# Ighina/MultimodalTopicSegmentation

Measured on NVIDIA B200. Metric: segmented sentences/sec, higher is better.
Workload: dtype f32

## Files before the change

### multimodaltopicsegmentation_b200/csrc/lstm_rec_h3.cu

```cuda
#include <cooperative_groups.h>
#include <cuda_fp16.h>
#include <stdlib.h>

#include "cluster_utils.cuh"
#include "tcgen05_utils.cuh"

namespace cg = cooperative_groups;

namespace mts {

constexpr int HR_NB = 16;
constexpr int HR_SUB_THREADS = 160;
constexpr int HR_EPI = 128;
constexpr int HR_PIECE_BYTES = 4 * HR_NB * 128;
constexpr int HR_B_BYTES = 2 * HR_PIECE_BYTES;
constexpr int HR_ACT_FLOATS = 4 * HR_NB * 32;
constexpr int HR_TMEM_COLS = 512;
constexpr int HR_W2_COL = 128;
constexpr int HR_ACC_COL = 256;
constexpr int HR_SUB_BYTES = 2 * HR_B_BYTES + HR_ACT_FLOATS * 4 + 1024;
constexpr int HR_HEAD_BYTES = 1024;
static_assert(HR_SUB_BYTES % 1024 == 0, "SWIZZLE_128B operand buffers need 1024-byte alignment");
template <int NT>
constexpr int hr_smem() {
  return (HR_HEAD_BYTES + NT * HR_SUB_BYTES + 1024) > 120 * 1024 ? (HR_HEAD_BYTES + NT * HR_SUB_BYTES + 1024) : 120 * 1024;
}

__host__ __device__ constexpr uint32_t idesc_f16(int M, int N) {
  return (1u << 4) | ((uint32_t)(N >> 3) << 17) | ((uint32_t)(M >> 4) << 24);
}

__device__ __forceinline__ uint32_t h2_bits(float first, float second) {
  const __half2 h = __floats2half2_rn(first, second);
  return *reinterpret_cast<const uint32_t *>(&h);
}
__device__ __forceinline__ float2 h2_floats(uint32_t bits) {
  return __half22float2(*reinterpret_cast<const __half2 *>(&bits));
}
__device__ __forceinline__ void st_async_v4u(uint32_t raddr, uint4 v, uint32_t rbar) {
  asm volatile("st.async.weak.shared::cluster.mbarrier::complete_tx::bytes.v4.b32 [%0], {%1, %2, %3, %4}, [%5];" ::"r"(raddr),
               "r"(v.x), "r"(v.y), "r"(v.z), "r"(v.w), "r"(rbar)
               : "memory");
}
__device__ __forceinline__ void tmem_st16u(uint32_t taddr, const uint32_t (&v)[16]) {
  asm volatile(
      "tcgen05.st.sync.aligned.32x32b.x16.b32 [%0], "
      "{%1, %2, %3, %4, %5, %6, %7, %8, %9, %10, %11, %12, %13, %14, %15, %16};" ::"r"(taddr),
      "r"(v[0]), "r"(v[1]), "r"(v[2]), "r"(v[3]), "r"(v[4]), "r"(v[5]), "r"(v[6]), "r"(v[7]), "r"(v[8]), "r"(v[9]), "r"(v[10]),
      "r"(v[11]), "r"(v[12]), "r"(v[13]), "r"(v[14]), "r"(v[15])
      : "memory");
}

__device__ __forceinline__ void umma_f16_ts_p(uint32_t d_tmem, uint32_t a_tmem, uint32_t b_lo, uint32_t b_hi, uint32_t idesc,
                                              uint32_t acc) {
  asm volatile(
      "{\n\t.reg .pred p;\n\t.reg .b64 bd;\n\t"
      "setp.ne.b32 p, %5, 0;\n\t"
      "mov.b64 bd, {%2, %3};\n\t"
      "tcgen05.mma.cta_group::1.kind::f16 [%0], [%1], bd, %4, p;\n\t}" ::"r"(d_tmem),
      "r"(a_tmem), "r"(b_lo), "r"(b_hi), "r"(idesc), "r"(acc)
      : "memory");
}

constexpr int HR_PROF_STEPS = 4, HR_PROF_SLOTS = 16;
__device__ long long *g_hr_prof = nullptr;
#define HR_STAMP(slot)                                                                     \
  do {                                                                                     \
    if (prof && s >= 8 && s < 8 + HR_PROF_STEPS) prof[(s - 8) * HR_PROF_SLOTS + (slot)] = clock64(); \
  } while (0)

template <bool SAVE, int NT, bool BF16>
__global__ void __cluster_dims__(kCluster, 1, 1) __launch_bounds__(HR_SUB_THREADS * NT, 1)
    lstm_fwd_h3_kernel(const float *__restrict__ gx, const float *__restrict__ w_hh, const int32_t *__restrict__ lengths,
                       const int32_t *__restrict__ order, int B, int T, int n_enc, int n_tiles, int ept,
                       float *__restrict__ y, float *__restrict__ gates, float *__restrict__ y_corr) {
  constexpr bool bf16_mode = BF16;
  extern __shared__ uint8_t smem_raw[];
  uint8_t *smem = reinterpret_cast<uint8_t *>((reinterpret_cast<uintptr_t>(smem_raw) + 1023) & ~(uintptr_t)1023);
  const int tid = threadIdx.x, lane = tid & 31;
  const int warp = __shfl_sync(0xffffffffu, tid >> 5, 0);
  const int sub = (NT == 2 && warp >= 5) ? 1 : 0;
  const int wr = warp - 5 * sub;

  float *rscale_s = reinterpret_cast<float *>(smem);
  uint32_t *tmem_slot = reinterpret_cast<uint32_t *>(smem + 512);
  uint8_t *sub_base = smem + HR_HEAD_BYTES + sub * HR_SUB_BYTES;
  uint8_t *bbuf = sub_base;
  float *act = reinterpret_cast<float *>(bbuf + 2 * HR_B_BYTES);
  uint64_t *bars = reinterpret_cast<uint64_t *>(act + HR_ACT_FLOATS);
  uint64_t *h_full = bars;
  uint64_t *acc_full = bars + 16;
  int *len_s = reinterpret_cast<int *>(bars + 18);
  int *bq_s = len_s + HR_NB;

  cg::cluster_group cluster = cg::this_cluster();
  const uint32_t rank = cluster.block_rank();
  const int n_clusters = gridDim.x / kCluster;
  const int groups = (n_tiles + NT - 1) / NT;
  const int n_items = groups * 2 * n_enc;
  const int ycols = n_enc * 2 * kH;

  if (wr == 0 && lane == 0) {
    for (int i = 0; i < 4; ++i) tc::bar_init(tc::s_u32(&h_full[i]), 1);
    tc::bar_init(tc::s_u32(acc_full), 1);
    asm volatile("fence.mbarrier_init.release.cluster;" ::: "memory");
  }
  if (warp == 0) tc::tmem_alloc<HR_TMEM_COLS>(tc::s_u32(tmem_slot));
  tc::tc_fence_before();
  __syncthreads();
  tc::tc_fence_after();
  const uint32_t tmem_base = *tmem_slot;
  const uint32_t acc_col = HR_ACC_COL + 16 * sub;

  uint32_t ph_h = 0, ph_acc = 0;

  const int et = (wr - 1) * 32 + lane;
  const int q = warp & 3;
  const int cj = et & 7, ce = et >> 3;

  int cur_dir = -1, cur_enc = -1;
  long long *prof = (blockIdx.x == 0 && (tid == 0 || tid == 32)) ? g_hr_prof : nullptr;

  for (int item = blockIdx.x / kCluster; item < n_items; item += n_clusters) {
    const int tile = (item % groups) * NT + sub;
    const int dir = (item / groups) & 1;
    const int enc = item / (2 * groups);
    const float *W = w_hh + ((size_t)enc * 2 + dir) * 4 * kH * kH;

    if (dir != cur_dir || enc != cur_enc) {
      if (sub == 0 && wr >= 1) {
        const float *wrow = W + (size_t)(q * kH + rank * kUnits + lane) * kH;
        float mx = 0.0f;
#pragma unroll 8
        for (int i = 0; i < kH / 4; ++i) {
          const float4 x = __ldg(reinterpret_cast<const float4 *>(wrow) + i);
          mx = fmaxf(fmaxf(mx, fmaxf(fabsf(x.x), fabsf(x.y))), fmaxf(fabsf(x.z), fabsf(x.w)));
        }
        const int ex = (int)((__float_as_uint(mx) >> 23) & 0xFFu);
        int sexp = ex == 0 ? 0 : 127 + 13 - ex;
        sexp = sexp > 110 ? 110 : sexp;
        const float sc = __uint_as_float((uint32_t)(127 + sexp) << 23);
        rscale_s[q * 32 + lane] = __uint_as_float((uint32_t)(127 - sexp) << 23);
        const uint32_t trow = tmem_base + ((uint32_t)(q * 32) << 16);
#pragma unroll 1
        for (int kk = 0; kk < 8; ++kk) {
          const int src_blk = ((int)rank - kk) & 7;
          uint32_t w1[16], w2[16];
#pragma unroll
          for (int i = 0; i < 8; ++i) {
            const float4 x = __ldg(reinterpret_cast<const float4 *>(wrow + src_blk * 32) + i);
            const float a = x.x * sc, b = x.y * sc, c = x.z * sc, d = x.w * sc;
            if (bf16_mode) {
              w1[2 * i] = bf16x2_bits(a, b);
              w1[2 * i + 1] = bf16x2_bits(c, d);
              w2[2 * i] = w2[2 * i + 1] = 0u;
            } else {
              w1[2 * i] = h2_bits(a, b);
              w1[2 * i + 1] = h2_bits(c, d);
              const float2 f0 = h2_floats(w1[2 * i]), f1 = h2_floats(w1[2 * i + 1]);
              w2[2 * i] = h2_bits(a - f0.x, b - f0.y);
              w2[2 * i + 1] = h2_bits(c - f1.x, d - f1.y);
            }
          }
          tmem_st16u(trow + (uint32_t)(kk * 16), w1);
          tmem_st16u(trow + (uint32_t)(HR_W2_COL + kk * 16), w2);
        }
        tc::tmem_wait_st();
      }
      cur_dir = dir;
      cur_enc = enc;
    }
    const int st = tid - sub * HR_SUB_THREADS;
    if (st < HR_NB) {
      const int slot = tile * ept + st;
      const int bq = (tile < n_tiles && st < ept && slot < B) ? (order ? order[slot] : slot) : -1;
      bq_s[st] = bq;
      len_s[st] = (bq >= 0) ? min(max(lengths[bq], 0), T) : 0;
    }
    for (int idx = st; idx < 2 * HR_B_BYTES / 16; idx += HR_SUB_THREADS)
      reinterpret_cast<float4 *>(bbuf)[idx] = make_float4(0.f, 0.f, 0.f, 0.f);
    tc::fence_proxy_async();
    tc::tc_fence_before();
    __syncthreads();
    tc::tc_fence_after();
    int nsteps = 0;
#pragma unroll
    for (int e = 0; e < HR_NB; ++e) nsteps = max(nsteps, len_s[e]);
    cluster.sync();

    const size_t gx_enc = (size_t)enc * B * T * 8 * kH;

    if (wr == 0) {
      constexpr uint32_t idesc = bf16_mode ? tc::idesc_bf16(128, HR_NB) : idesc_f16(128, HR_NB);
      const uint32_t tb = __shfl_sync(0xffffffffu, tmem_base, 0);
      const uint32_t d_tmem = tb + acc_col;
      const bool leader = tc::elect_one();
      const uint64_t dfull = tc::desc_sw128(tc::s_u32(bbuf));
      const uint32_t dlo0 = __shfl_sync(0xffffffffu, (uint32_t)dfull, 0), dhi = (uint32_t)(dfull >> 32);
      const uint32_t half_tx = (uint32_t)(4 * ept * (bf16_mode ? 64 : 128));
      for (int s = 0; s < nsteps; ++s) {
        const int p = s & 1;
        HR_STAMP(0);
        if (leader && s + 1 < nsteps) {
          tc::bar_expect_tx(tc::s_u32(&h_full[(p ^ 1) * 2 + 0]), half_tx);
          tc::bar_expect_tx(tc::s_u32(&h_full[(p ^ 1) * 2 + 1]), half_tx);
        }
        const uint32_t dlo = dlo0 + (uint32_t)(p * (HR_B_BYTES >> 4));
#pragma unroll
        for (int g = 0; g < 2; ++g) {
          if (s > 0) tc::bar_wait_wd(tc::s_u32(&h_full[p * 2 + g]), (ph_h >> p) & 1u);
          HR_STAMP(1 + g);
          tc::tc_fence_after();
          if (leader) {
#pragma unroll
            for (int i = 4 * g; i < 4 * g + 4; ++i) {
#pragma unroll
              for (int k = 0; k < 2; ++k) {
                const uint32_t d1 = dlo + (uint32_t)(((i >> 1) * (HR_NB * 128) + (i & 1) * 64 + k * 32) >> 4);
                const uint32_t d2 = d1 + (uint32_t)(HR_PIECE_BYTES >> 4);
                const uint32_t a1 = tb + (uint32_t)(16 * i + 8 * k), a2 = a1 + HR_W2_COL;
                umma_f16_ts_p(d_tmem, a1, d1, dhi, idesc, (i | k) != 0);
                if (!bf16_mode) {
                  umma_f16_ts_p(d_tmem, a2, d1, dhi, idesc, 1);
                  umma_f16_ts_p(d_tmem, a1, d2, dhi, idesc, 1);
                }
              }
            }
          }
          HR_STAMP(3 + g);
        }
        if (s > 0) ph_h ^= 1u << p;
        if (leader) tc::umma_commit(tc::s_u32(acc_full));
        __syncwarp();
        HR_STAMP(5);
      }
    } else {
      const int gcol = dir * 4 * kH + q * kH + (int)rank * kUnits + lane;
      const float rs = rscale_s[q * 32 + lane];
      float gxn[HR_NB];
#pragma unroll
      for (int e = 0; e < HR_NB; ++e) {
        const int len = len_s[e];
        gxn[e] = 0.0f;
        if (len > 0) {
          const int t0 = dir ? len - 1 : 0;
          gxn[e] = __ldg(gx + gx_enc + ((size_t)bq_s[e] * T + t0) * 8 * kH + gcol);
        }
      }
      float c[4] = {0.f, 0.f, 0.f, 0.f};
      const int my_len = len_s[ce], my_b = bq_s[ce];
      const size_t ycol = (size_t)enc * 2 * kH + dir * kH + rank * kUnits + 4 * cj;
      const size_t gate_base = ((size_t)enc * 2 + dir) * B;
      const int piece = cj & 1, chunk = cj >> 1;
      uint32_t raddr[kCluster], rbar[kCluster];
#pragma unroll
      for (int i = 0; i < kCluster; ++i) {
        const uint32_t r = (rank + i) & 7;
        const uint32_t off = (uint32_t)(piece * HR_PIECE_BYTES + (i >> 1) * (HR_NB * 128) + ce * 128 +
                                        ((((i & 1) * 4 + chunk) ^ (ce & 7)) << 4));
        raddr[i] = mapa(tc::s_u32(bbuf) + off, r);
        rbar[i] = mapa(tc::s_u32(&h_full[i >> 2]), r);
      }
      const bool sender = ce < ept && !(bf16_mode && piece);

      for (int s = 0; s < nsteps; ++s) {
        const int p = s & 1;
        float gxc[HR_NB];
#pragma unroll
        for (int e = 0; e < HR_NB; ++e) {
          gxc[e] = gxn[e];
          const int len = len_s[e];
          if (s + 1 < len) {
            const int tn = dir ? len - 2 - s : s + 1;
            gxn[e] = __ldg(gx + gx_enc + ((size_t)bq_s[e] * T + tn) * 8 * kH + gcol);
          }
        }
        tc::bar_wait_wd(tc::s_u32(acc_full), ph_acc); ph_acc ^= 1;
        HR_STAMP(10);
        tc::tc_fence_after();
        float pre[HR_NB];
        tc::tmem_ld16(tmem_base + ((uint32_t)(q * 32) << 16) + acc_col, pre);
        tc::tc_fence_before();
        HR_STAMP(11);
        const float zs = (q == 2) ? -2.0f * 1.4426950408889634f : -1.4426950408889634f;
        const float oa = (q == 2) ? 2.0f : 1.0f, ob = (q == 2) ? -1.0f : 0.0f;
#define HR_ACT(NCOL)                                                          \
  _Pragma("unroll") for (int e = 0; e < (NCOL); ++e) {                        \
    const float z = fmaf(pre[e], rs, gxc[e]);                                 \
    const float sg = __fdividef(1.0f, 1.0f + exp2f(z * zs));                  \
    act[(q * HR_NB + e) * 32 + lane] = fmaf(sg, oa, ob);                      \
  }
        if (ept > 14) { HR_ACT(16) } else if (ept > 12) { HR_ACT(14) } else if (ept > 10) { HR_ACT(12) } else if (ept > 8) { HR_ACT(10) }
        else if (ept > 6) { HR_ACT(8) } else if (ept > 4) { HR_ACT(6) } else if (ept > 2) { HR_ACT(4) } else { HR_ACT(2) }
#undef HR_ACT
        if (sub == 0) asm volatile("bar.sync 1, 128;" ::: "memory");
        else asm volatile("bar.sync 2, 128;" ::: "memory");
        HR_STAMP(12);
        const float4 ig = *reinterpret_cast<const float4 *>(act + (0 * HR_NB + ce) * 32 + 4 * cj);
        const float4 fg = *reinterpret_cast<const float4 *>(act + (1 * HR_NB + ce) * 32 + 4 * cj);
        const float4 gg = *reinterpret_cast<const float4 *>(act + (2 * HR_NB + ce) * 32 + 4 * cj);
        const float4 og = *reinterpret_cast<const float4 *>(act + (3 * HR_NB + ce) * 32 + 4 * cj);
        float4 hn = make_float4(0.f, 0.f, 0.f, 0.f);
        if (s < my_len) {
          c[0] = fmaf(fg.x, c[0], ig.x * gg.x); c[1] = fmaf(fg.y, c[1], ig.y * gg.y);
          c[2] = fmaf(fg.z, c[2], ig.z * gg.z); c[3] = fmaf(fg.w, c[3], ig.w * gg.w);
          hn = make_float4(og.x * tanh_fast(c[0]), og.y * tanh_fast(c[1]), og.z * tanh_fast(c[2]), og.w * tanh_fast(c[3]));
        }
        HR_STAMP(13);
        if (s + 1 < nsteps) {
          uint32_t p1a, p1b, p2a = 0u, p2b = 0u;
          if (bf16_mode) {
            p1a = bf16x2_bits(hn.x, hn.y);
            p1b = bf16x2_bits(hn.z, hn.w);
          } else {
            p1a = h2_bits(hn.x, hn.y);
            p1b = h2_bits(hn.z, hn.w);
            const float2 f0 = h2_floats(p1a), f1 = h2_floats(p1b);
            p2a = h2_bits(hn.x - f0.x, hn.y - f0.y);
            p2b = h2_bits(hn.z - f1.x, hn.w - f1.y);
          }
          const uint32_t ga = piece ? p1a : p2a, gb = piece ? p1b : p2b;
          const uint32_t ra = __shfl_xor_sync(0xffffffffu, ga, 1), rb = __shfl_xor_sync(0xffffffffu, gb, 1);
          const uint4 gran = piece ? make_uint4(ra, rb, p2a, p2b) : make_uint4(p1a, p1b, ra, rb);
          if (sender) {
            const uint32_t boff = (uint32_t)((p ^ 1) * HR_B_BYTES), moff = (uint32_t)((p ^ 1) * 16);
#pragma unroll
            for (int r = 0; r < kCluster; ++r) st_async_v4u(raddr[r] + boff, gran, rbar[r] + moff);
          }
        }
        HR_STAMP(14);
        if (s < my_len) {
          const int t = dir ? my_len - 1 - s : s;
          *reinterpret_cast<float4 *>(y + ((size_t)my_b * T + t) * ycols + ycol) = hn;
          if (y_corr) corr_store4(y_corr + ((size_t)my_b * T + t) * ycols, (int)ycol, hn, 0);
          if (SAVE) {
            float *gs = gates + ((gate_base + my_b) * T + t) * 5 * kH + rank * kUnits + 4 * cj;
            *reinterpret_cast<float4 *>(gs) = ig;
            *reinterpret_cast<float4 *>(gs + kH) = fg;
            *reinterpret_cast<float4 *>(gs + 2 * kH) = gg;
            *reinterpret_cast<float4 *>(gs + 3 * kH) = og;
            *reinterpret_cast<float4 *>(gs + 4 * kH) = make_float4(c[0], c[1], c[2], c[3]);
          }
        }
      }
      if (my_b >= 0)
        for (int t = my_len; t < T; ++t) {
          const float4 z = make_float4(0.f, 0.f, 0.f, 0.f);
          *reinterpret_cast<float4 *>(y + ((size_t)my_b * T + t) * ycols + ycol) = z;
          if (y_corr) corr_store4(y_corr + ((size_t)my_b * T + t) * ycols, (int)ycol, z, 0);
        }
    }
    tc::tc_fence_before();
    __syncthreads();
    cluster.sync();
  }
  tc::tc_fence_before();
  __syncthreads();
  if (warp == 0) {
    tc::tc_fence_after();
    tc::tmem_dealloc<HR_TMEM_COLS>(tmem_base);
  }
}

template <typename K>
static int h3_max_active_clusters(K kernel, int threads, int smem) {
  cudaLaunchConfig_t cfg = {};
  cfg.gridDim = dim3(kCluster * 64);
  cfg.blockDim = dim3(threads);
  cfg.dynamicSmemBytes = smem;
  cudaLaunchAttribute attr;
  attr.id = cudaLaunchAttributeClusterDimension;
  attr.val.clusterDim.x = kCluster;
  attr.val.clusterDim.y = 1;
  attr.val.clusterDim.z = 1;
  cfg.attrs = &attr;
  cfg.numAttrs = 1;
  int n = 0;
  if (cudaOccupancyMaxActiveClusters(&n, kernel, &cfg) != cudaSuccess || n < 1) {
    cudaGetLastError();
    n = 8;
  }
  return n;
}

}

using namespace mts;

extern "C" int mts_debug_rec_profile_h3(long long *buf) {
  MTS_CUDA(cudaMemcpyToSymbol(g_hr_prof, &buf, sizeof(buf)));
  return 0;
}

template <bool BF16>
static int launch_h3(const float *gx, const float *w_hh, const int32_t *lengths, const int32_t *order, int n_enc, int B, int T,
                     float *y, float *gates, float *y_corr, cudaStream_t st) {
  MTS_PER_DEVICE(int, cap);
  if (!cap) {
    MTS_CUDA(cudaFuncSetAttribute(lstm_fwd_h3_kernel<false, 1, BF16>, cudaFuncAttributeMaxDynamicSharedMemorySize, hr_smem<1>()));
    MTS_CUDA(cudaFuncSetAttribute(lstm_fwd_h3_kernel<true, 1, BF16>, cudaFuncAttributeMaxDynamicSharedMemorySize, hr_smem<1>()));
    MTS_CUDA(cudaFuncSetAttribute(lstm_fwd_h3_kernel<false, 2, BF16>, cudaFuncAttributeMaxDynamicSharedMemorySize, hr_smem<2>()));
    MTS_CUDA(cudaFuncSetAttribute(lstm_fwd_h3_kernel<true, 2, BF16>, cudaFuncAttributeMaxDynamicSharedMemorySize, hr_smem<2>()));
    cap = h3_max_active_clusters(lstm_fwd_h3_kernel<false, 2, BF16>, 2 * HR_SUB_THREADS, hr_smem<2>());
  }
  int ept = HR_NB;
  {
    const int per_dir = cap / (2 * n_enc);
    if (per_dir >= 1 && (B + HR_NB - 1) / HR_NB <= per_dir) {
      const int want = (B + per_dir - 1) / per_dir;
      ept = want < 1 ? 1 : (want > HR_NB ? HR_NB : want);
    }
  }
  static const char *force_ept = getenv("MTS_REC_EPT");
  if (force_ept && atoi(force_ept) >= 1 && atoi(force_ept) <= HR_NB) ept = atoi(force_ept);
  const int n_tiles = (B + ept - 1) / ept;
  const int items1 = n_tiles * 2 * n_enc;
  static const char *force = getenv("MTS_REC_NT");
  const bool two = force ? (force[0] == '2') : (items1 > cap);
  static const char *pair_env = getenv("MTS_REC_PAIR");
  if (pair_env ? (pair_env[0] == '1') : two)
    return mts_lstm_rec_fwd_h3p(gx, w_hh, lengths, order, n_enc, B, T, kH, y, gates, y_corr, BF16 ? 1 : 0, (void *)st);
  if (!two) {
    const unsigned grid = (unsigned)((items1 < cap ? items1 : cap) * kCluster);
    if (gates) lstm_fwd_h3_kernel<true, 1, BF16><<<grid, HR_SUB_THREADS, hr_smem<1>(), st>>>(gx, w_hh, lengths, order, B, T, n_enc, n_tiles, ept, y, gates, y_corr);
    else lstm_fwd_h3_kernel<false, 1, BF16><<<grid, HR_SUB_THREADS, hr_smem<1>(), st>>>(gx, w_hh, lengths, order, B, T, n_enc, n_tiles, ept, y, gates, y_corr);
  } else {
    const int items2 = ((n_tiles + 1) / 2) * 2 * n_enc;
    const unsigned grid = (unsigned)((items2 < cap ? items2 : cap) * kCluster);
    if (gates) lstm_fwd_h3_kernel<true, 2, BF16><<<grid, 2 * HR_SUB_THREADS, hr_smem<2>(), st>>>(gx, w_hh, lengths, order, B, T, n_enc, n_tiles, ept, y, gates, y_corr);
    else lstm_fwd_h3_kernel<false, 2, BF16><<<grid, 2 * HR_SUB_THREADS, hr_smem<2>(), st>>>(gx, w_hh, lengths, order, B, T, n_enc, n_tiles, ept, y, gates, y_corr);
  }
  MTS_LAUNCH_CHECK();
  return 0;
}

extern "C" int mts_lstm_rec_fwd_h3(const float *gx, const float *w_hh, const int32_t *lengths, const int32_t *order, int n_enc,
                                   int B, int T, int H, float *y, float *gates, float *y_corr, int precision, void *stream) {
  MTS_REQUIRE(gx && w_hh && lengths && y, MTS_E_BADARG, "lstm_rec_fwd_h3: null pointer");
  MTS_REQUIRE(n_enc >= 1 && B > 0 && T > 0, MTS_E_BADARG, "lstm_rec_fwd_h3: bad shape");
  MTS_REQUIRE(H == kH, MTS_E_UNSUPPORTED, "lstm_rec_fwd_h3: the tensor-core recurrence serves H == 256");
  MTS_REQUIRE(precision == 0 || precision == 1, MTS_E_BADARG, "lstm_rec_fwd_h3: precision must be 0 (fp16 x3) or 1 (bf16)");
  MTS_REQUIRE(!y_corr || n_enc == 1, MTS_E_UNSUPPORTED, "lstm_rec_fwd_h3: the fused correction operand needs n_enc == 1");
  MTS_REQUIRE((((uintptr_t)y | (uintptr_t)gx | (uintptr_t)w_hh) & 15) == 0, MTS_E_BADARG,
              "lstm_rec_fwd_h3: buffers must be 16-byte aligned");
  cudaStream_t st = (cudaStream_t)stream;
  return precision ? launch_h3<true>(gx, w_hh, lengths, order, n_enc, B, T, y, gates, y_corr, st)
                   : launch_h3<false>(gx, w_hh, lengths, order, n_enc, B, T, y, gates, y_corr, st);
}
```

Before: 18.96 million.

## Widen single-tile LSTM recurrence kernel to eight epilogue warps splitting batch columns

For the one-tile-per-CTA launch, the kernel now runs 288 threads. Eight epilogue warps split the 16 batch columns into two halves, and each thread owns two hidden units instead of four. Gate loads use incrementing pointers, the TMEM accumulator load is halved, the sigmoid uses a raw ex2.approx, and the h broadcast is regrouped with an extra shuffle stage. The goal is to shorten the per-step serial latency of the recurrence at the cost of more threads, extra shuffles and a wider barrier.

```diff
diff --git a/multimodaltopicsegmentation_b200/csrc/lstm_rec_h3.cu b/multimodaltopicsegmentation_b200/csrc/lstm_rec_h3.cu
--- a/multimodaltopicsegmentation_b200/csrc/lstm_rec_h3.cu
+++ b/multimodaltopicsegmentation_b200/csrc/lstm_rec_h3.cu
@@ -11,7 +11,7 @@
 
 constexpr int HR_NB = 16;
 constexpr int HR_SUB_THREADS = 160;
-constexpr int HR_EPI = 128;
+constexpr int HR_WIDE_THREADS = 288;
 constexpr int HR_PIECE_BYTES = 4 * HR_NB * 128;
 constexpr int HR_B_BYTES = 2 * HR_PIECE_BYTES;
 constexpr int HR_ACT_FLOATS = 4 * HR_NB * 32;
@@ -42,6 +42,23 @@
                "r"(v.x), "r"(v.y), "r"(v.z), "r"(v.w), "r"(rbar)
                : "memory");
 }
+__device__ __forceinline__ void tmem_ld8(uint32_t taddr, float (&v)[8]) {
+  uint32_t r[8];
+  asm volatile("tcgen05.ld.sync.aligned.32x32b.x8.b32 {%0, %1, %2, %3, %4, %5, %6, %7}, [%8];"
+               : "=r"(r[0]), "=r"(r[1]), "=r"(r[2]), "=r"(r[3]), "=r"(r[4]), "=r"(r[5]), "=r"(r[6]), "=r"(r[7])
+               : "r"(taddr)
+               : "memory");
+  asm volatile("tcgen05.wait::ld.sync.aligned;" ::: "memory");
+#pragma unroll
+  for (int i = 0; i < 8; ++i) v[i] = __uint_as_float(r[i]);
+}
+__device__ __forceinline__ int hr_col_of_slot(int e) { return (e & 1) * 8 + (e >> 1); }
+__device__ __forceinline__ int hr_slot_of_col(int c) { return (c & 7) * 2 + (c >> 3); }
+__device__ __forceinline__ float ex2_ftz(float x) {
+  float y;
+  asm("ex2.approx.ftz.f32 %0, %1;" : "=f"(y) : "f"(x));
+  return y;
+}
 __device__ __forceinline__ void tmem_st16u(uint32_t taddr, const uint32_t (&v)[16]) {
   asm volatile(
       "tcgen05.st.sync.aligned.32x32b.x16.b32 [%0], "
@@ -70,11 +87,13 @@
   } while (0)
 
 template <bool SAVE, int NT, bool BF16>
-__global__ void __cluster_dims__(kCluster, 1, 1) __launch_bounds__(HR_SUB_THREADS * NT, 1)
+__global__ void __cluster_dims__(kCluster, 1, 1) __launch_bounds__(NT == 1 ? HR_WIDE_THREADS : HR_SUB_THREADS * NT, 1)
     lstm_fwd_h3_kernel(const float *__restrict__ gx, const float *__restrict__ w_hh, const int32_t *__restrict__ lengths,
                        const int32_t *__restrict__ order, int B, int T, int n_enc, int n_tiles, int ept,
                        float *__restrict__ y, float *__restrict__ gates, float *__restrict__ y_corr) {
   constexpr bool bf16_mode = BF16;
+  constexpr bool WIDE = NT == 1;
+  constexpr int PIPE_THREADS = WIDE ? HR_WIDE_THREADS : HR_SUB_THREADS;
   extern __shared__ uint8_t smem_raw[];
   uint8_t *smem = reinterpret_cast<uint8_t *>((reinterpret_cast<uintptr_t>(smem_raw) + 1023) & ~(uintptr_t)1023);
   const int tid = threadIdx.x, lane = tid & 31;
@@ -116,7 +135,9 @@
 
   const int et = (wr - 1) * 32 + lane;
   const int q = warp & 3;
-  const int cj = et & 7, ce = et >> 3;
+  const int half = WIDE ? (wr - 1) >> 2 : 0;
+  constexpr int CU = WIDE ? 2 : 4;
+  const int cj = WIDE ? (et & 15) : (et & 7), ce = WIDE ? (et >> 4) : (et >> 3);
 
   int cur_dir = -1, cur_enc = -1;
   long long *prof = (blockIdx.x == 0 && (tid == 0 || tid == 32)) ? g_hr_prof : nullptr;
@@ -128,7 +149,7 @@
     const float *W = w_hh + ((size_t)enc * 2 + dir) * 4 * kH * kH;
 
     if (dir != cur_dir || enc != cur_enc) {
-      if (sub == 0 && wr >= 1) {
+      if (sub == 0 && wr >= 1 && (!WIDE || wr <= 4)) {
         const float *wrow = W + (size_t)(q * kH + rank * kUnits + lane) * kH;
         float mx = 0.0f;
 #pragma unroll 8
@@ -172,12 +193,13 @@
     }
     const int st = tid - sub * HR_SUB_THREADS;
     if (st < HR_NB) {
-      const int slot = tile * ept + st;
-      const int bq = (tile < n_tiles && st < ept && slot < B) ? (order ? order[slot] : slot) : -1;
+      const int es = WIDE ? hr_slot_of_col(st) : st;
+      const int slot = tile * ept + es;
+      const int bq = (tile < n_tiles && es < ept && slot < B) ? (order ? order[slot] : slot) : -1;
       bq_s[st] = bq;
       len_s[st] = (bq >= 0) ? min(max(lengths[bq], 0), T) : 0;
     }
-    for (int idx = st; idx < 2 * HR_B_BYTES / 16; idx += HR_SUB_THREADS)
+    for (int idx = st; idx < 2 * HR_B_BYTES / 16; idx += PIPE_THREADS)
       reinterpret_cast<float4 *>(bbuf)[idx] = make_float4(0.f, 0.f, 0.f, 0.f);
     tc::fence_proxy_async();
     tc::tc_fence_before();
@@ -235,51 +257,72 @@
         HR_STAMP(5);
       }
     } else {
+      constexpr int NG = WIDE ? HR_NB / 2 : HR_NB;
+      const int gc0 = 8 * half;
       const int gcol = dir * 4 * kH + q * kH + (int)rank * kUnits + lane;
       const float rs = rscale_s[q * 32 + lane];
-      float gxn[HR_NB];
-#pragma unroll
-      for (int e = 0; e < HR_NB; ++e) {
-        const int len = len_s[e];
+      float gxn[NG];
+      int glen[WIDE ? NG : 1];
+      const float *gptr[WIDE ? NG : 1];
+      const ptrdiff_t gstep = dir ? -8 * kH : 8 * kH;
+#pragma unroll
+      for (int e = 0; e < NG; ++e) {
+        const int len = len_s[gc0 + e];
         gxn[e] = 0.0f;
+        if constexpr (WIDE) { glen[e] = len; gptr[e] = gx; }
         if (len > 0) {
           const int t0 = dir ? len - 1 : 0;
-          gxn[e] = __ldg(gx + gx_enc + ((size_t)bq_s[e] * T + t0) * 8 * kH + gcol);
+          const float *gp = gx + gx_enc + ((size_t)bq_s[gc0 + e] * T + t0) * 8 * kH + gcol;
+          if constexpr (WIDE) gptr[e] = gp;
+          gxn[e] = __ldg(gp);
         }
       }
-      float c[4] = {0.f, 0.f, 0.f, 0.f};
-      const int my_len = len_s[ce], my_b = bq_s[ce];
-      const size_t ycol = (size_t)enc * 2 * kH + dir * kH + rank * kUnits + 4 * cj;
+      float c[CU];
+#pragma unroll
+      for (int u = 0; u < CU; ++u) c[u] = 0.0f;
+      const int ccol = WIDE ? hr_col_of_slot(ce) : ce;
+      const int my_len = len_s[ccol], my_b = bq_s[ccol];
+      const size_t ycol = (size_t)enc * 2 * kH + dir * kH + rank * kUnits + CU * cj;
       const size_t gate_base = ((size_t)enc * 2 + dir) * B;
-      const int piece = cj & 1, chunk = cj >> 1;
-      uint32_t raddr[kCluster], rbar[kCluster];
-#pragma unroll
-      for (int i = 0; i < kCluster; ++i) {
+      const int piece = (WIDE && bf16_mode) ? 0 : (cj & 1), chunk = WIDE ? cj >> 2 : cj >> 1;
+      constexpr int NDST = WIDE ? (bf16_mode ? 2 : 4) : kCluster;
+      uint32_t raddr[NDST], rbar[NDST];
+#pragma unroll
+      for (int m = 0; m < NDST; ++m) {
+        const int i = !WIDE ? m : bf16_mode ? 4 * m + (cj & 3) : 2 * m + ((cj >> 1) & 1);
         const uint32_t r = (rank + i) & 7;
-        const uint32_t off = (uint32_t)(piece * HR_PIECE_BYTES + (i >> 1) * (HR_NB * 128) + ce * 128 +
-                                        ((((i & 1) * 4 + chunk) ^ (ce & 7)) << 4));
-        raddr[i] = mapa(tc::s_u32(bbuf) + off, r);
-        rbar[i] = mapa(tc::s_u32(&h_full[i >> 2]), r);
+        const uint32_t off = (uint32_t)(piece * HR_PIECE_BYTES + (i >> 1) * (HR_NB * 128) + ccol * 128 +
+                                        ((((i & 1) * 4 + chunk) ^ (ccol & 7)) << 4));
+        raddr[m] = mapa(tc::s_u32(bbuf) + off, r);
+        rbar[m] = mapa(tc::s_u32(&h_full[i >> 2]), r);
       }
-      const bool sender = ce < ept && !(bf16_mode && piece);
+      const bool sender = ce < ept && !(!WIDE && bf16_mode && piece);
 
       for (int s = 0; s < nsteps; ++s) {
         const int p = s & 1;
-        float gxc[HR_NB];
-#pragma unroll
-        for (int e = 0; e < HR_NB; ++e) {
+        float gxc[NG];
+#pragma unroll
+        for (int e = 0; e < NG; ++e) {
           gxc[e] = gxn[e];
-          const int len = len_s[e];
-          if (s + 1 < len) {
-            const int tn = dir ? len - 2 - s : s + 1;
-            gxn[e] = __ldg(gx + gx_enc + ((size_t)bq_s[e] * T + tn) * 8 * kH + gcol);
+          if constexpr (WIDE) {
+            if (s + 1 < glen[e]) {
+              gptr[e] += gstep;
+              gxn[e] = __ldg(gptr[e]);
+            }
+          } else {
+            const int len = len_s[gc0 + e];
+            if (s + 1 < len) {
+              const int tn = dir ? len - 2 - s : s + 1;
+              gxn[e] = __ldg(gx + gx_enc + ((size_t)bq_s[gc0 + e] * T + tn) * 8 * kH + gcol);
+            }
           }
         }
         tc::bar_wait_wd(tc::s_u32(acc_full), ph_acc); ph_acc ^= 1;
         HR_STAMP(10);
         tc::tc_fence_after();
-        float pre[HR_NB];
-        tc::tmem_ld16(tmem_base + ((uint32_t)(q * 32) << 16) + acc_col, pre);
+        float pre[NG];
+        if constexpr (WIDE) tmem_ld8(tmem_base + ((uint32_t)(q * 32) << 16) + acc_col + gc0, pre);
+        else tc::tmem_ld16(tmem_base + ((uint32_t)(q * 32) << 16) + acc_col, pre);
         tc::tc_fence_before();
         HR_STAMP(11);
         const float zs = (q == 2) ? -2.0f * 1.4426950408889634f : -1.4426950408889634f;
@@ -287,67 +330,134 @@
 #define HR_ACT(NCOL)                                                          \
   _Pragma("unroll") for (int e = 0; e < (NCOL); ++e) {                        \
     const float z = fmaf(pre[e], rs, gxc[e]);                                 \
-    const float sg = __fdividef(1.0f, 1.0f + exp2f(z * zs));                  \
-    act[(q * HR_NB + e) * 32 + lane] = fmaf(sg, oa, ob);                      \
-  }
-        if (ept > 14) { HR_ACT(16) } else if (ept > 12) { HR_ACT(14) } else if (ept > 10) { HR_ACT(12) } else if (ept > 8) { HR_ACT(10) }
-        else if (ept > 6) { HR_ACT(8) } else if (ept > 4) { HR_ACT(6) } else if (ept > 2) { HR_ACT(4) } else { HR_ACT(2) }
+    const float sg = __fdividef(1.0f, 1.0f + (WIDE ? ex2_ftz(z * zs) : exp2f(z * zs)));  \
+    act[(q * HR_NB + gc0 + e) * 32 + lane] = fmaf(sg, oa, ob);                \
+  }
+        if constexpr (WIDE) {
+          switch ((ept + 1) >> 1) {
+            case 1: HR_ACT(1) break;
+            case 2: HR_ACT(2) break;
+            case 3: HR_ACT(3) break;
+            case 4: HR_ACT(4) break;
+            case 5: HR_ACT(5) break;
+            case 6: HR_ACT(6) break;
+            case 7: HR_ACT(7) break;
+            default: HR_ACT(8) break;
+          }
+          asm volatile("bar.sync 1, 256;" ::: "memory");
+        } else {
+          if (ept > 14) { HR_ACT(16) } else if (ept > 12) { HR_ACT(14) } else if (ept > 10) { HR_ACT(12) } else if (ept > 8) { HR_ACT(10) }
+          else if (ept > 6) { HR_ACT(8) } else if (ept > 4) { HR_ACT(6) } else if (ept > 2) { HR_ACT(4) } else { HR_ACT(2) }
+          if (sub == 0) asm volatile("bar.sync 1, 128;" ::: "memory");
+          else asm volatile("bar.sync 2, 128;" ::: "memory");
+        }
 #undef HR_ACT
-        if (sub == 0) asm volatile("bar.sync 1, 128;" ::: "memory");
-        else asm volatile("bar.sync 2, 128;" ::: "memory");
         HR_STAMP(12);
-        const float4 ig = *reinterpret_cast<const float4 *>(act + (0 * HR_NB + ce) * 32 + 4 * cj);
-        const float4 fg = *reinterpret_cast<const float4 *>(act + (1 * HR_NB + ce) * 32 + 4 * cj);
-        const float4 gg = *reinterpret_cast<const float4 *>(act + (2 * HR_NB + ce) * 32 + 4 * cj);
-        const float4 og = *reinterpret_cast<const float4 *>(act + (3 * HR_NB + ce) * 32 + 4 * cj);
-        float4 hn = make_float4(0.f, 0.f, 0.f, 0.f);
-        if (s < my_len) {
-          c[0] = fmaf(fg.x, c[0], ig.x * gg.x); c[1] = fmaf(fg.y, c[1], ig.y * gg.y);
-          c[2] = fmaf(fg.z, c[2], ig.z * gg.z); c[3] = fmaf(fg.w, c[3], ig.w * gg.w);
-          hn = make_float4(og.x * tanh_fast(c[0]), og.y * tanh_fast(c[1]), og.z * tanh_fast(c[2]), og.w * tanh_fast(c[3]));
-        }
-        HR_STAMP(13);
-        if (s + 1 < nsteps) {
-          uint32_t p1a, p1b, p2a = 0u, p2b = 0u;
-          if (bf16_mode) {
-            p1a = bf16x2_bits(hn.x, hn.y);
-            p1b = bf16x2_bits(hn.z, hn.w);
-          } else {
-            p1a = h2_bits(hn.x, hn.y);
-            p1b = h2_bits(hn.z, hn.w);
-            const float2 f0 = h2_floats(p1a), f1 = h2_floats(p1b);
-            p2a = h2_bits(hn.x - f0.x, hn.y - f0.y);
-            p2b = h2_bits(hn.z - f1.x, hn.w - f1.y);
-          }
-          const uint32_t ga = piece ? p1a : p2a, gb = piece ? p1b : p2b;
-          const uint32_t ra = __shfl_xor_sync(0xffffffffu, ga, 1), rb = __shfl_xor_sync(0xffffffffu, gb, 1);
-          const uint4 gran = piece ? make_uint4(ra, rb, p2a, p2b) : make_uint4(p1a, p1b, ra, rb);
-          if (sender) {
-            const uint32_t boff = (uint32_t)((p ^ 1) * HR_B_BYTES), moff = (uint32_t)((p ^ 1) * 16);
-#pragma unroll
-            for (int r = 0; r < kCluster; ++r) st_async_v4u(raddr[r] + boff, gran, rbar[r] + moff);
-          }
-        }
-        HR_STAMP(14);
-        if (s < my_len) {
-          const int t = dir ? my_len - 1 - s : s;
-          *reinterpret_cast<float4 *>(y + ((size_t)my_b * T + t) * ycols + ycol) = hn;
-          if (y_corr) corr_store4(y_corr + ((size_t)my_b * T + t) * ycols, (int)ycol, hn, 0);
-          if (SAVE) {
-            float *gs = gates + ((gate_base + my_b) * T + t) * 5 * kH + rank * kUnits + 4 * cj;
-            *reinterpret_cast<float4 *>(gs) = ig;
-            *reinterpret_cast<float4 *>(gs + kH) = fg;
-            *reinterpret_cast<float4 *>(gs + 2 * kH) = gg;
-            *reinterpret_cast<float4 *>(gs + 3 * kH) = og;
-            *reinterpret_cast<float4 *>(gs + 4 * kH) = make_float4(c[0], c[1], c[2], c[3]);
+        if constexpr (WIDE) {
+          const float2 ig = *reinterpret_cast<const float2 *>(act + (0 * HR_NB + ccol) * 32 + 2 * cj);
+          const float2 fg = *reinterpret_cast<const float2 *>(act + (1 * HR_NB + ccol) * 32 + 2 * cj);
+          const float2 gg = *reinterpret_cast<const float2 *>(act + (2 * HR_NB + ccol) * 32 + 2 * cj);
+          const float2 og = *reinterpret_cast<const float2 *>(act + (3 * HR_NB + ccol) * 32 + 2 * cj);
+          float2 hn = make_float2(0.f, 0.f);
+          if (s < my_len) {
+            c[0] = fmaf(fg.x, c[0], ig.x * gg.x); c[1] = fmaf(fg.y, c[1], ig.y * gg.y);
+            hn = make_float2(og.x * tanh_fast(c[0]), og.y * tanh_fast(c[1]));
+          }
+          HR_STAMP(13);
+          if (s + 1 < nsteps) {
+            uint32_t p1, p2 = 0u;
+            if (bf16_mode) {
+              p1 = bf16x2_bits(hn.x, hn.y);
+            } else {
+              p1 = h2_bits(hn.x, hn.y);
+              const float2 f0 = h2_floats(p1);
+              p2 = h2_bits(hn.x - f0.x, hn.y - f0.y);
+            }
+            const uint32_t mine = piece ? p2 : p1;
+            const uint32_t r = __shfl_xor_sync(0xffffffffu, (bf16_mode || piece) ? p1 : p2, 1);
+            const uint32_t w0 = (cj & 1) ? r : mine, w1 = (cj & 1) ? mine : r;
+            const uint32_t x0 = __shfl_xor_sync(0xffffffffu, w0, 2), x1 = __shfl_xor_sync(0xffffffffu, w1, 2);
+            const uint4 gran = (cj & 2) ? make_uint4(x0, x1, w0, w1) : make_uint4(w0, w1, x0, x1);
+            if (sender) {
+              const uint32_t boff = (uint32_t)((p ^ 1) * HR_B_BYTES), moff = (uint32_t)((p ^ 1) * 16);
+#pragma unroll
+              for (int m = 0; m < NDST; ++m) st_async_v4u(raddr[m] + boff, gran, rbar[m] + moff);
+            }
+          }
+          HR_STAMP(14);
+          if (s < my_len) {
+            const int t = dir ? my_len - 1 - s : s;
+            *reinterpret_cast<float2 *>(y + ((size_t)my_b * T + t) * ycols + ycol) = hn;
+            if (y_corr) corr_store2(y_corr + ((size_t)my_b * T + t) * ycols, (int)ycol, hn, 0);
+            if (SAVE) {
+              float *gs = gates + ((gate_base + my_b) * T + t) * 5 * kH + rank * kUnits + 2 * cj;
+              *reinterpret_cast<float2 *>(gs) = ig;
+              *reinterpret_cast<float2 *>(gs + kH) = fg;
+              *reinterpret_cast<float2 *>(gs + 2 * kH) = gg;
+              *reinterpret_cast<float2 *>(gs + 3 * kH) = og;
+              *reinterpret_cast<float2 *>(gs + 4 * kH) = make_float2(c[0], c[1]);
+            }
+          }
+        } else {
+          const float4 ig = *reinterpret_cast<const float4 *>(act + (0 * HR_NB + ce) * 32 + 4 * cj);
+          const float4 fg = *reinterpret_cast<const float4 *>(act + (1 * HR_NB + ce) * 32 + 4 * cj);
+          const float4 gg = *reinterpret_cast<const float4 *>(act + (2 * HR_NB + ce) * 32 + 4 * cj);
+          const float4 og = *reinterpret_cast<const float4 *>(act + (3 * HR_NB + ce) * 32 + 4 * cj);
+          float4 hn = make_float4(0.f, 0.f, 0.f, 0.f);
+          if (s < my_len) {
+            c[0] = fmaf(fg.x, c[0], ig.x * gg.x); c[1] = fmaf(fg.y, c[1], ig.y * gg.y);
+            c[2] = fmaf(fg.z, c[2], ig.z * gg.z); c[3] = fmaf(fg.w, c[3], ig.w * gg.w);
+            hn = make_float4(og.x * tanh_fast(c[0]), og.y * tanh_fast(c[1]), og.z * tanh_fast(c[2]), og.w * tanh_fast(c[3]));
+          }
+          HR_STAMP(13);
+          if (s + 1 < nsteps) {
+            uint32_t p1a, p1b, p2a = 0u, p2b = 0u;
+            if (bf16_mode) {
+              p1a = bf16x2_bits(hn.x, hn.y);
+              p1b = bf16x2_bits(hn.z, hn.w);
+            } else {
+              p1a = h2_bits(hn.x, hn.y);
+              p1b = h2_bits(hn.z, hn.w);
+              const float2 f0 = h2_floats(p1a), f1 = h2_floats(p1b);
+              p2a = h2_bits(hn.x - f0.x, hn.y - f0.y);
+              p2b = h2_bits(hn.z - f1.x, hn.w - f1.y);
+            }
+            const uint32_t ga = piece ? p1a : p2a, gb = piece ? p1b : p2b;
+            const uint32_t ra = __shfl_xor_sync(0xffffffffu, ga, 1), rb = __shfl_xor_sync(0xffffffffu, gb, 1);
+            const uint4 gran = piece ? make_uint4(ra, rb, p2a, p2b) : make_uint4(p1a, p1b, ra, rb);
+            if (sender) {
+              const uint32_t boff = (uint32_t)((p ^ 1) * HR_B_BYTES), moff = (uint32_t)((p ^ 1) * 16);
+#pragma unroll
+              for (int r = 0; r < kCluster; ++r) st_async_v4u(raddr[r] + boff, gran, rbar[r] + moff);
+            }
+          }
+          HR_STAMP(14);
+          if (s < my_len) {
+            const int t = dir ? my_len - 1 - s : s;
+            *reinterpret_cast<float4 *>(y + ((size_t)my_b * T + t) * ycols + ycol) = hn;
+            if (y_corr) corr_store4(y_corr + ((size_t)my_b * T + t) * ycols, (int)ycol, hn, 0);
+            if (SAVE) {
+              float *gs = gates + ((gate_base + my_b) * T + t) * 5 * kH + rank * kUnits + 4 * cj;
+              *reinterpret_cast<float4 *>(gs) = ig;
+              *reinterpret_cast<float4 *>(gs + kH) = fg;
+              *reinterpret_cast<float4 *>(gs + 2 * kH) = gg;
+              *reinterpret_cast<float4 *>(gs + 3 * kH) = og;
+              *reinterpret_cast<float4 *>(gs + 4 * kH) = make_float4(c[0], c[1], c[2], c[3]);
+            }
           }
         }
       }
       if (my_b >= 0)
         for (int t = my_len; t < T; ++t) {
-          const float4 z = make_float4(0.f, 0.f, 0.f, 0.f);
-          *reinterpret_cast<float4 *>(y + ((size_t)my_b * T + t) * ycols + ycol) = z;
-          if (y_corr) corr_store4(y_corr + ((size_t)my_b * T + t) * ycols, (int)ycol, z, 0);
+          if constexpr (WIDE) {
+            const float2 z = make_float2(0.f, 0.f);
+            *reinterpret_cast<float2 *>(y + ((size_t)my_b * T + t) * ycols + ycol) = z;
+            if (y_corr) corr_store2(y_corr + ((size_t)my_b * T + t) * ycols, (int)ycol, z, 0);
+          } else {
+            const float4 z = make_float4(0.f, 0.f, 0.f, 0.f);
+            *reinterpret_cast<float4 *>(y + ((size_t)my_b * T + t) * ycols + ycol) = z;
+            if (y_corr) corr_store4(y_corr + ((size_t)my_b * T + t) * ycols, (int)ycol, z, 0);
+          }
         }
     }
     tc::tc_fence_before();
@@ -422,8 +532,8 @@
     return mts_lstm_rec_fwd_h3p(gx, w_hh, lengths, order, n_enc, B, T, kH, y, gates, y_corr, BF16 ? 1 : 0, (void *)st);
   if (!two) {
     const unsigned grid = (unsigned)((items1 < cap ? items1 : cap) * kCluster);
-    if (gates) lstm_fwd_h3_kernel<true, 1, BF16><<<grid, HR_SUB_THREADS, hr_smem<1>(), st>>>(gx, w_hh, lengths, order, B, T, n_enc, n_tiles, ept, y, gates, y_corr);
-    else lstm_fwd_h3_kernel<false, 1, BF16><<<grid, HR_SUB_THREADS, hr_smem<1>(), st>>>(gx, w_hh, lengths, order, B, T, n_enc, n_tiles, ept, y, gates, y_corr);
+    if (gates) lstm_fwd_h3_kernel<true, 1, BF16><<<grid, HR_WIDE_THREADS, hr_smem<1>(), st>>>(gx, w_hh, lengths, order, B, T, n_enc, n_tiles, ept, y, gates, y_corr);
+    else lstm_fwd_h3_kernel<false, 1, BF16><<<grid, HR_WIDE_THREADS, hr_smem<1>(), st>>>(gx, w_hh, lengths, order, B, T, n_enc, n_tiles, ept, y, gates, y_corr);
   } else {
     const int items2 = ((n_tiles + 1) / 2) * 2 * n_enc;
     const unsigned grid = (unsigned)((items2 < cap ? items2 : cap) * kCluster);
```

After: 18.42 million, median of 6. 2.8% lower.
